# DanecLacey/basic_iterative_solvers

Measured on AMD Instinct MI355X. Metric: CG iterations/sec + SpMV GFLOP/s (% HBM roofline), HPCG 256^3 at 1/2/4/8 GPUs, higher is better.
Workload: dtype f64

## Files before the change

### basic_iterative_solvers_amd/csrc/bis_blas1.hip

```cpp
#include "bis_internal.hpp"

#include <algorithm>
#include <cstdlib>

namespace {

constexpr int kEwThreads = 256;
constexpr int kMaxEwBlocks = 16384;

inline int ew_grid(int64_t n_items) {
    int64_t g = (n_items + kEwThreads - 1) / kEwThreads;
    if (g < 1) g = 1;
    if (g > kMaxDotBlocks) g = kMaxDotBlocks;
    return (int)g;
}
inline int ew_grid_wide(int64_t n_items) {
    int64_t g = (n_items + kEwThreads - 1) / kEwThreads;
    if (g < 1) g = 1;
    if (g > kMaxEwBlocks) g = kMaxEwBlocks;
    return (int)g;
}

typedef double ew_v2d_t __attribute__((ext_vector_type(2)));
__device__ __forceinline__ double2 ld_stream(const double2 *p) {
// ... 180 lines not shown
}

}

bis_status bis_reduce_finish(bis_ctx *ctx, int n_partials, int n_values, size_t stride,
                             double *result_dev) {
    hipLaunchKernelGGL(reduce_finish_kernel, dim3(n_values), dim3(256), 0, ctx->stream,
                       ctx->partials, n_partials, stride, result_dev);
    BIS_HIP_CHECK(ctx, hipGetLastError());
    return BIS_OK;
}

bis_status bis_ensure_partials(bis_ctx *ctx, size_t n) {
    if (n <= ctx->partials_cap) return BIS_OK;
    BIS_HIP_CHECK(ctx, hipStreamSynchronize(ctx->stream));
    if (ctx->partials) BIS_HIP_CHECK(ctx, hipFree(ctx->partials));
    ctx->partials = nullptr;
    ctx->partials_cap = 0;
    BIS_HIP_CHECK(ctx, hipMalloc(&ctx->partials, sizeof(double) * n));
    ctx->partials_cap = n;
    return BIS_OK;
}

bis_status bis_fault_check(bis_ctx *ctx) {
    volatile unsigned *f = ctx->fault_host;
    if (!f || *f == 0) return BIS_OK;
    *f = 0;
    ctx->err = "a triangular sweep lost a hand-off: a row waited for a result that was never published "
               "(a workgroup of the persistent grid could not become resident, or the dependency data is corrupt); "
               "the vectors written since the last blocking call are invalid";
    return BIS_ERR_SYNC;
}

#define BIS_OPTIONS_ENV(X) X(spmv_variant) X(spmv_window) X(spmv_chunk) X(spmv_chunk_fused) X(spmv_xcd_remap) X(trsv_grid) X(ilu0_wgs) X(trsv_wave_wgs) X(trsv_trial) X(trsv_one_xcd) X(trsv_host_analysis) X(ilu0_wave) X(spmv_packed) X(spmv_packed32) X(spmv_valdict) X(spmv_sellwin) X(device_share) X(spmv_sellwin_rows) X(spmv_sellwin_joint) X(spmv_sellwin_pairs) X(spmv_sellwin_masks) X(spmv_colslab) X(spmv_win8) X(spmv_win8_rows) X(spmv_win8_depth) X(spmv_win8_implicit) X(spmv_win8_tune) X(grid_autodetect) X(tune_placement) X(force_rp64) X(trsv_tiled) X(trsv_chain) X(trsv_tile_rows) X(trsv_tile_wgs) X(trsv_tile_edge) X(trsv_tile_backoff)
#define BIS_OPTIONS_API(Y) Y(trsv_batch) Y(trsv_wave) Y(ilu0_persistent) Y(trsv_by_pos) Y(spmv_lds_pad) Y(trsv_chain_idle) Y(trsv_chain_pause) Y(trsv_chain_pairs) Y(trsv_chain_prefix) Y(trsv_tile_exp) Y(cg_nt_x) Y(spmv_sellwin_nt) Y(dist_host_plan) Y(trsv_inject_loss) Y(trsv_inject_oom)

namespace {
std::string &opts_env_seen() { static std::string s; return s; }
std::string upper_env(const char *name) {
    std::string e = "BIS_";
    for (const char *c = name; *c; ++c) e += (char)((*c >= 'a' && *c <= 'z') ? *c - 32 : *c);
    return e;
}
}

bis_options &bis_opts() {
    static bis_options o = [] {
        bis_options v;
#define X(name) { const std::string en = upper_env(#name); if (const char *e = getenv(en.c_str())) { v.name = atoi(e); \
                  std::string &seen = opts_env_seen(); if (!seen.empty()) seen += ' '; seen += en + "=" + e; } }
        BIS_OPTIONS_ENV(X)
#undef X
        return v;
    }();
    return o;
}

extern "C" {

bis_status bis_set_option(const char *name, int value) {
    if (!name) return BIS_ERR_INVALID;
    bis_options &o = bis_opts();
#define X(opt) if (!strcmp(name, #opt)) { o.opt = value; return BIS_OK; }
    BIS_OPTIONS_ENV(X)
    BIS_OPTIONS_API(X)
#undef X
    return BIS_ERR_INVALID;
// ... 377 lines not shown
```

### basic_iterative_solvers_amd/csrc/bis_internal.hpp

```cpp
#pragma once

#include <hip/hip_runtime.h>

#include <cstdint>
#include <cstdio>
#include <cstring>
#include <map>
#include <string>
#include <vector>

#include "bis_hip.h"

struct bis_trsv_plan;

struct bis_named_kernel {
    int type = 0;
    const bis_mat *A = nullptr;
    double *B = nullptr, *C = nullptr;
    int64_t size_B = 0, size_C = 0;
    const double *D = nullptr;
    bool upper = false;
};

struct bis_ctx {
// ... 41 lines not shown
    int trsv_trial = -1;
    int trsv_batch = -1;
    int trsv_by_pos = -1;
    int trsv_one_xcd = -1;
    int tune_placement = -1;
    int spmv_packed32 = -1;
    int spmv_lds_pad = -1;
    int spmv_packed = -1;
    int spmv_valdict = -1;
    int dist_host_plan = -1;
    int grid_autodetect = -1;
    int trsv_chain = -1;
    int trsv_chain_idle = -1;
    int trsv_chain_pause = -1;
    int trsv_chain_prefix = -1;
    int trsv_chain_pairs = -1;
    int trsv_tiled = -1;
    int trsv_tile_rows = -1;
    int trsv_tile_wgs = -1;
    int trsv_tile_backoff = -1;
    int spmv_sellwin_nt = -1;
    int cg_nt_x = -1;
    int trsv_tile_exp = -1;
    int trsv_tile_edge = -1;
    int force_rp64 = -1;
    int spmv_sellwin = -1;
    int spmv_sellwin_rows = -1;
    int spmv_sellwin_pairs = -1;
    int spmv_sellwin_joint = -1;
    int spmv_colslab = -1;
    int spmv_win8 = -1;
    int spmv_win8_rows = -1;
    int spmv_win8_depth = -1;
    int spmv_win8_implicit = -1;
    int spmv_win8_tune = -1;
    int spmv_sellwin_masks = -1;
    int device_share = -1;
    int trsv_inject_oom = -1;
    int trsv_inject_loss = -1;
};
inline bool bis_want_rp64(int64_t nnz) { return nnz >= (int64_t)INT32_MAX - 8 || bis_opts().force_rp64 > 0; }

constexpr int kMaxReduceBlocks = 2048;
constexpr int kMaxDotBlocks = 8192;
constexpr int kWinMaxTiles = 128;
constexpr int kWinTile = 16;
constexpr int kWinTileLog = 4;
constexpr int kSwRows = 256;
constexpr int kSwMaxR = 4;

struct bis_mat {
    int64_t n_rows = 0, n_cols = 0, nnz = 0;
    bool rp64 = false;
    bool view = false;
    void *row_ptr = nullptr;
    int32_t *col = nullptr;
    double *val = nullptr;
    int32_t *blk_row = nullptr;
    int64_t *blk_nnz = nullptr;
    uint16_t *loc = nullptr;
    int32_t *tiles = nullptr;
    int32_t *tile_cnt = nullptr;
    int64_t loc_base = 0;
    int max_tiles = 0;
    bool win_ok = false;
    int n_blocks = 0;
// ... 115 lines not shown
    ++ctx->prof_used;
}

bis_status bis_reduce_finish(bis_ctx *ctx, int n_partials, int n_values,
                             size_t stride, double *result_dev);
bis_status bis_ensure_partials(bis_ctx *ctx, size_t n);
bis_status bis_spmv_launch(bis_ctx *ctx, const bis_mat *A, const double *x,
                           double *y, const double *w, int *n_partials,
                           size_t partials_off = 0);
size_t bis_spmv_partials_bound(const bis_mat *A);
bis_status bis_spmv_trsv_level(bis_ctx *ctx, const bis_mat *T, const double *x, double *y,
                               const double *b, const double *D);
bis_status bis_mat_row_view(bis_ctx *ctx, const bis_mat *A, int64_t ra,
                            int64_t rb, bis_mat **out);

bis_status bis_mat_alloc(bis_ctx *ctx, int64_t n_rows, int64_t n_cols,
                         int64_t nnz, bool rp64, bis_mat **out);
bis_status bis_mat_finalize(bis_ctx *ctx, bis_mat *A);
bis_status bis_spmv_build_window(bis_ctx *ctx, bis_mat *A);
void bis_spmv_drop_packed(bis_mat *A);
void bis_spmv_drop_valdict(bis_mat *A);
bis_status bis_spmv_try_valdict(bis_ctx *ctx, bis_mat *A, bool consecutive_ok);
bis_status bis_spmv_sellwin_try(bis_ctx *ctx, bis_mat *A);
int bis_spmv_sellwin_blocks(const bis_mat *A);
int64_t bis_spmv_sellwin_bytes(const bis_mat *A);
int64_t bis_spmv_sellwin_slices(const bis_mat *A);
int bis_spmv_sellwin_format(const bis_mat *A);
bis_status bis_spmv_sellwin_launch(bis_ctx *ctx, const bis_mat *A, const double *x, double *y, int mode, const double *w,
                                   double *partials, const int *stop, int remap_arg, int grid);
void bis_spmv_sellwin_drop(bis_mat *A);
bis_status bis_spmv_win8_try(bis_ctx *ctx, bis_mat *A);
int bis_spmv_win8_blocks(const bis_mat *A);
int bis_spmv_win8_rows(const bis_mat *A);
int64_t bis_spmv_win8_bytes(const bis_mat *A);
bis_status bis_spmv_win8_launch(bis_ctx *ctx, const bis_mat *A, const double *x, double *y, int mode, const double *w,
                                double *partials, const int *stop, int remap_arg, int grid);
void bis_spmv_win8_drop(bis_mat *A);
bis_status bis_spmv_colslab_build(bis_ctx *ctx, const bis_mat *A, int K, std::vector<bis_mat *> &slabs, bool *ok);
void bis_spmv_colslab_free(bis_ctx *ctx, std::vector<bis_mat *> &slabs);
void bis_spmv_colslab_drop(bis_mat *A);
int bis_spmv_remap_arg(int nb);
int bis_spmv_grid(int nb);
size_t bis_spmv_win8_stream_bytes(const bis_mat *A);
bool bis_spmv_win8_implied(const bis_mat *A);
double bis_spmv_win8_moved_bytes(const bis_mat *A);
bool bis_spmv_win8_fast(const bis_mat *A, double ms);
void *bis_spmv_win8_swap_stream(bis_mat *A, void *stream);
bis_status bis_spmv_try_pack(bis_ctx *ctx, bis_mat *A, int t);
void bis_mat_free_meta(bis_mat *A);
void bis_mat_values_changed(bis_mat *A);
void bis_trsv_plan_destroy(bis_trsv_plan *p);
void bis_trsv_plan_adopt(bis_mat *to, bis_mat *from, bool backward);
bis_status bis_mat_split_strict_impl(bis_ctx *ctx, const bis_mat *A, bis_mat **L_strict,
                                     bis_mat **U_strict, double *D, double *D_inv, bool check_diag);
struct bis_trsv_tiled;
bis_status bis_trsv_tiled_build(bis_ctx *ctx, const bis_mat *T, bool backward, bis_trsv_tiled **out);
bis_status bis_trsv_tiled_solve(bis_ctx *ctx, bis_trsv_tiled *p, double *x, const double *D, const double *b);
void bis_trsv_tiled_destroy(bis_trsv_tiled *p);
bis_status bis_trsv_analyse_device(bis_ctx *ctx, const bis_mat *T, bool backward, int32_t *perm_dev,
                                   std::vector<int64_t> &level_ptr, int &n_levels, int64_t &max_width,
                                   bool &triangular, int **level_out = nullptr);
struct bis_trsv_chain;
bis_status bis_trsv_chain_build(bis_ctx *ctx, const bis_mat *T, bool backward, const int *level_dev, int n_levels,
                                bis_trsv_chain **out);
bis_status bis_trsv_chain_solve(bis_ctx *ctx, const bis_mat *T, bis_trsv_chain *p, double *x, const double *D, const double *b);
void bis_trsv_chain_destroy(bis_trsv_chain *p);
// ... 6 lines not shown
```

### basic_iterative_solvers_amd/csrc/bis_spmv.hip

```cpp
#include "bis_internal.hpp"

#include <algorithm>
#include <cstdlib>
#include <vector>

namespace {

typedef int v4i __attribute__((ext_vector_type(4)));
typedef double v2d __attribute__((ext_vector_type(2)));

typedef unsigned short v4us __attribute__((ext_vector_type(4)));

template <bool WIDE>
__device__ __forceinline__ double x_at(const char *xb, int c) {
    if (WIDE) return *reinterpret_cast<const double *>(xb + (int64_t)c * 8);
    return *reinterpret_cast<const double *>(xb + (uint32_t)((uint32_t)c << 3));
}

constexpr int kPkSegs = 8, kPkOffBits = 13, kPkSpan = 1 << kPkOffBits;
constexpr int kPk3Segs = 32, kPk3OffBits = 11;

template <int PK>
__device__ __forceinline__ int pk_decode(unsigned code, const int (&B)[8], int lane_base, int col_max) {
    int base;
// ... 755 lines not shown
int grid_for_map(int nb, int remap_arg) {
    const int w = remap_arg < -1 ? 8 * -remap_arg : 8;
    return (nb + w - 1) / w * w;
}

int fused_threads(int) { return 256; }

int spmv_variant(const SpmvArgs &a) {
    const int v = bis_opts().spmv_variant >= 0 ? bis_opts().spmv_variant : (a.pk_mode ? 20 : 41);
    return (a.pk_mode >= 2 && v % 10 != 0) ? 20 : v;
}

const char *rowblock_name(int id, const SpmvArgs &a) {
    static const std::vector<std::string> names = [] {
        std::vector<std::string> v;
        for (int u : {1, 2, 4})
            for (int pk = 0; pk < 5; ++pk)
                for (int br = 0; br < 3; ++br)
                    v.push_back("spmv_rowblock_kernel U=" + std::to_string(u) + " PK=" + (pk == 4 ? std::string("0 WIDE") : std::to_string(pk)) +
                                " BR=" + std::to_string(br));
        return v;
    }();
    if (rowblock_is_vd(id, a)) return "spmv_rowblock_vd_kernel";
    const int u = id / 10 == 1 ? 0 : (id / 10 == 2 ? 1 : 2), br = id % 10;
    static const int known[] = {10, 20, 40, 11, 21, 41, 12, 22};
    if (std::find(std::begin(known), std::end(known), id) == std::end(known)) return nullptr;
    const int pk = a.wide ? 4 : a.pk_mode;
    return names[(size_t)(u * 5 + pk) * 3 + br].c_str();
}

const char *form_name(int kind, int v) {
    static const std::vector<std::string> names[3] = {
        [] { std::vector<std::string> n; for (int i = 0; i <= 4; ++i) n.push_back("sellwin fmt=" + std::to_string(i)); return n; }(),
        [] { std::vector<std::string> n; for (int i = 0; i <= 4; ++i) n.push_back("win8 rows=" + std::to_string(i)); return n; }(),
        [] { std::vector<std::string> n; for (int i = 0; i <= 32; ++i) n.push_back("colslab K=" + std::to_string(i)); return n; }()};
    const std::vector<std::string> &t = names[kind];
    return t[(size_t)std::max(0, std::min(v, (int)t.size() - 1))].c_str();
}

}

int spmv_window_mode() { return bis_opts().spmv_window < 0 ? 0 : bis_opts().spmv_window; }

bis_status bis_spmv_build_window(bis_ctx *ctx, bis_mat *A) {
    A->win_ok = false;
    if (!spmv_window_mode() || A->nnz == 0 || A->n_rows == 0) return BIS_OK;
    if ((int64_t)A->chunk_nnz + A->max_row_nnz + 8 > 6144) return BIS_OK;
    const int nb = A->n_blocks;
    int64_t ends[2];
    BIS_HIP_CHECK(ctx, hipMemcpyAsync(&ends[0], A->blk_nnz, 8, hipMemcpyDeviceToHost, ctx->stream));
    BIS_HIP_CHECK(ctx, hipMemcpyAsync(&ends[1], A->blk_nnz + nb, 8, hipMemcpyDeviceToHost, ctx->stream));
    BIS_HIP_CHECK(ctx, hipStreamSynchronize(ctx->stream));
    A->loc_base = ends[0] & ~(int64_t)3;
    const size_t n_loc = (size_t)(ends[1] - A->loc_base) + 16;
    hipFree(A->loc); hipFree(A->tiles); hipFree(A->tile_cnt);
    A->loc = nullptr; A->tiles = nullptr; A->tile_cnt = nullptr;
    BIS_HIP_CHECK(ctx, hipMalloc(&A->loc, sizeof(uint16_t) * n_loc));
    BIS_HIP_CHECK(ctx, hipMalloc(&A->tiles, sizeof(int32_t) * (size_t)nb * kWinMaxTiles));
    BIS_HIP_CHECK(ctx, hipMalloc(&A->tile_cnt, sizeof(int32_t) * (size_t)nb));
    BIS_HIP_CHECK(ctx, hipMemsetAsync(A->loc, 0, sizeof(uint16_t) * n_loc, ctx->stream));
    int *status = (int *)ctx->counters + 40;
    BIS_HIP_CHECK(ctx, hipMemsetAsync(status, 0, 2 * sizeof(int), ctx->stream));
    if (A->rp64)
        hipLaunchKernelGGL(window_build_kernel<int64_t>, dim3(nb), dim3(256), 0, ctx->stream, A->col,
                           A->blk_nnz, nb, A->loc_base, A->loc, A->tiles, A->tile_cnt, status);
    else
        hipLaunchKernelGGL(window_build_kernel<int32_t>, dim3(nb), dim3(256), 0, ctx->stream, A->col,
// ... 378 lines not shown
    }
    if (bis_status st = ensure_packed(ctx, A, use_f ? 1 : 0, &a)) return st;
    if (pass) {
        a.vcode = nullptr;
    } else {
        const int v = bis_opts().spmv_variant;
        const bool lane_per_row = a.vcode && spmv_valdict_mode() >= 2 && (v < 0 || v == 20);
        if (mode != 2 && lane_per_row && bis_opts().spmv_sellwin != 0) {
            if (bis_status st = bis_spmv_sellwin_try(ctx, A)) return st;
            if (const int nb = bis_spmv_sellwin_blocks(A)) {
                block_map(nb);
                p->form = kFormSellwin;
                p->n_partials = mode == 1 ? (int)bis_spmv_sellwin_slices(A) : 0;
                p->name = form_name(0, bis_spmv_sellwin_format(A));
                return BIS_OK;
            }
        }
        if (lane_per_row) {
            if (bis_status st = spmv_try_rowmajor(ctx, A)) return st;
            if (A->rm_state == 1) {
                block_map(A->rm_blocks);
                p->form = kFormRowmajor;
                p->n_partials = mode == 1 ? A->rm_blocks * 4 : 0;
                p->name = "spmv_rowmajor_vd_kernel";
                return BIS_OK;
            }
        }
        if (mode != 2 && !a.vcode && bis_opts().spmv_win8 != 0 && (v < 0 || v == 20)) {
            if (bis_status st = bis_spmv_win8_try(ctx, A)) return st;
            if (const int nb = bis_spmv_win8_blocks(A)) {
                block_map(nb);
                p->form = kFormWin8;
                p->n_partials = mode == 1 ? nb * 4 : 0;
                p->name = form_name(1, bis_spmv_win8_rows(A));
                return BIS_OK;
            }
        }
        if (mode != 2 && !a.vcode && !a.wide && bis_opts().spmv_colslab != 0 && (v < 0 || v == 20 || v == 41)) {
            if (bis_status st = colslab_try(ctx, A, a.pk_mode != 0)) return st;
            if (A->cs_state == 1) {
                p->form = kFormColslab;
                p->n_partials = mode == 1 ? A->colslabs->back()->n_blocks_f * (fused_threads(0) / 64) : 0;
                p->name = form_name(2, (int)A->colslabs->size());
                return BIS_OK;
            }
        }
        if (mode != 2 && bis_opts().spmv_lds_pad > 0) a.lds_bytes += (size_t)bis_opts().spmv_lds_pad;
    }
    const int id = spmv_variant(a);
    p->name = rowblock_name(id, a);
    if (!p->name) { ctx->err = "bis_spmv: unknown BIS_SPMV_VARIANT"; return BIS_ERR_INVALID; }
    p->form = rowblock_is_vd(id, a) ? kFormRowblockVd : kFormRowblock;
    p->n_partials = mode == 1 ? a.nb * (fused_threads(id) / 64) : 0;
    return BIS_OK;
}

static bis_status spmv_launch_plan(bis_ctx *ctx, const bis_mat *A, const SpmvPlan &p) {
    const SpmvArgs &a = p.a;
    switch (p.form) {
    case kFormLongRows: {
        const int grid = (int)std::min<int64_t>((A->n_rows + 3) / 4, 8192);
        if (A->rp64)
            hipLaunchKernelGGL(spmv_wave_per_row_kernel<int64_t>, dim3(grid), dim3(256), 0, ctx->stream,
                               (const int64_t *)A->row_ptr, A->col, A->val, a.x, a.y, A->n_rows);
        else
            hipLaunchKernelGGL(spmv_wave_per_row_kernel<int32_t>, dim3(grid), dim3(256), 0, ctx->stream,
                               (const int32_t *)A->row_ptr, A->col, A->val, a.x, a.y, A->n_rows);
// ... 189 lines not shown
```

### basic_iterative_solvers_amd/csrc/bis_spmv_sell.hip

```cpp
#include <algorithm>
#include <cstring>
#include <cstdio>
#include <cstdlib>
#include <vector>

#include <rocprim/rocprim.hpp>

#include "bis_internal.hpp"

struct bis_sellwin {
    int n_blocks = 0;
    int64_t n_slices = 0, total_chunks = 0;
    int32_t *hdr = nullptr;
    int64_t *slice_chunk0 = nullptr;
    int32_t *own_rank = nullptr;
    uint32_t *codes = nullptr;
    double *dict = nullptr;
    int max_gran = 0;
    int fmt = 0;
    int uniform_chunks = 0;
    int n_pairs = 0, pair_stride = 0, diag_pair = -1;
    int16_t *blk_base = nullptr;
    unsigned long long *pair_key = nullptr;
    uint16_t *row_of = nullptr;
    void *own_codes = nullptr;
    size_t w8_desc = 0, w8_side = 0, w8_end = 0;
    int64_t *slice_rec = nullptr;
    int64_t expl_chunks = 0;
    int64_t win_gran_sum = 0;
    int tune_trials = 0;
    double tune_first_ms = 0.0, tune_kept_ms = 0.0;
    int R = 1;
    bool diag = false;
    int pad_idx = 0, diag_idx = 0;
};

namespace {

constexpr int kSwRuns = 32;
constexpr int kSwRunGran = 64;
constexpr int kSwHash = 4096;
constexpr int kSwMaxGran = 940;
constexpr int kSwDefaultR = 2;
constexpr int kSwMaxPairs = 253;
inline int sw_gran_cap(int R) { return R == 4 ? kSwMaxGran : std::min(kSwMaxGran, (65536 - (4096 + 4096 * R) - 16) / 64); }

__device__ __forceinline__ unsigned long long sw_pair_key(int32_t offset, unsigned vcode) {
    return ((unsigned long long)((unsigned)offset ^ 0x80000000u) << 8) | vcode;
}

__device__ __forceinline__ int sw_wave_max(int v) {
    for (int o = 32; o > 0; o >>= 1) v = max(v, __shfl_xor(v, o));
    return v;
}

template <typename RP>
__global__ __launch_bounds__(256) void sw_plan_kernel(const RP *__restrict__ row_ptr, const int32_t *__restrict__ col,
                                                      int64_t n_rows, int R, int max_gran, int64_t row0, int32_t *__restrict__ hdr,
                                                      int32_t *__restrict__ slice_chunks, int32_t *__restrict__ own_rank, int *status) {
    __shared__ int table[kSwHash];
    __shared__ int list[1024];
// ... 1167 lines not shown
            if ((c_first & 7) == 0 && g0 <= g_first && g_last <= g1) own = rank + (g_first - g0);
            for (int o = 0; o < len && ok; o += kSwRunGran) {
                if (m >= kW8Runs) { ok = false; break; }
                out_g0[m] = g0 + o;
                out_rk[m] = (rank + o) | (min(kSwRunGran, len - o) << 16);
                ++m;
            }
            rank += len;
            if (rank > max_gran) ok = false;
        }
        if (!ok) atomicExch(&failed, 1);
        n_out = m;
        win_gran = rank;
        own_s = own;
    }
    __syncthreads();
    if (failed) {
        if (tid == 0) atomicExch(&status[0], 1);
        return;
    }
    if (tid < 2 * kW8Runs) {
        const int k = tid % kW8Runs;
        int word = 0;
        if (k < n_out) word = tid < kW8Runs ? out_g0[k] : out_rk[k];
        hdr[(size_t)b * 2 * kW8Runs + tid] = word;
    }
    if (tid == 0) {
        own_rank[b] = ident ? own_s : -1;
        atomicMax(&status[1], win_gran);
        atomicAdd(reinterpret_cast<unsigned *>(&status[2]), (unsigned)win_gran);
    }
}

template <typename RP, int PHASE>
__global__ __launch_bounds__(256) void w8_fill_kernel(const RP *__restrict__ row_ptr, const int32_t *__restrict__ col, const double *__restrict__ val,
                                                      int64_t n_rows, int R, const int32_t *__restrict__ hdr,
                                                      const int64_t *__restrict__ slice_chunk0, const uint16_t *__restrict__ row_of,
                                                      unsigned char *__restrict__ stream, int64_t *__restrict__ slice_rec,
                                                      uint2 *__restrict__ desc, unsigned char *__restrict__ side) {
    __shared__ int g0s[kW8Runs], rk[kW8Runs];
    __shared__ int nr_s;
    const int b = blockIdx.x, tid = threadIdx.x, lane = tid & 63, wv = tid >> 6;
    if (tid < kW8Runs) {
        g0s[tid] = hdr[(size_t)b * 2 * kW8Runs + tid];
        const int w2 = hdr[(size_t)b * 2 * kW8Runs + kW8Runs + tid];
        rk[tid] = w2 & 0xffff;
        const unsigned long long m = __ballot((w2 >> 16) != 0);
        if (tid == 0) nr_s = __popcll(m);
    }
    __syncthreads();
    const int nr = nr_s;
    for (int rr = 0; rr < R; ++rr) {
        const int64_t slice = ((int64_t)b * 4 + wv) * R + rr;
        const int64_t pos = slice * 64 + lane;
        const int in_block = row_of[pos];
        const int64_t r = (int64_t)b * kSwRows * R + in_block;
        int64_t rs = 0;
        int len = 0;
        if (r < n_rows) {
            rs = (int64_t)row_ptr[r];
            len = (int)((int64_t)row_ptr[r + 1] - rs);
        }
        const int64_t c0 = slice_chunk0[slice];
        const int nch = (int)(slice_chunk0[slice + 1] - c0);
        bool implicit = false;
        if (PHASE == 1) implicit = __ballot(r < n_rows && len == __builtin_amdgcn_readfirstlane(len)) == ~0ull;
// ... 50 lines not shown
    const unsigned char *p = stream + (size_t)c * kW8ChunkBytes;
    W8Chunk ch;
    ch.code = __builtin_nontemporal_load(reinterpret_cast<const w8_v2u *>(p + lane * 8));
    ch.v0 = __builtin_nontemporal_load(reinterpret_cast<const w8_v2d *>(p + 512 + lane * 16));
    ch.v1 = __builtin_nontemporal_load(reinterpret_cast<const w8_v2d *>(p + 1536 + lane * 16));
    return ch;
}

__device__ __forceinline__ void w8_load_values(const unsigned char *__restrict__ stream, int64_t c, int lane, W8Chunk &ch) {
    const unsigned char *p = stream + (size_t)c * kW8ValBytes;
    ch.v0 = __builtin_nontemporal_load(reinterpret_cast<const w8_v2d *>(p + lane * 16));
    ch.v1 = __builtin_nontemporal_load(reinterpret_cast<const w8_v2d *>(p + 1024 + lane * 16));
}

typedef unsigned short w8_v2h __attribute__((ext_vector_type(2)));
__device__ __forceinline__ unsigned w8_imply(unsigned code, unsigned off2) {
    const unsigned pad = (code & 0x10001u) * 0xffffu;
    return __builtin_bit_cast(unsigned, __builtin_bit_cast(w8_v2h, code) + __builtin_bit_cast(w8_v2h, off2)) & ~pad;
}

__device__ __forceinline__ void w8_consume(const unsigned char *win, const W8Chunk &ch, double &acc) {
#pragma clang fp contract(off)
    const double x0 = *reinterpret_cast<const double *>(win + (ch.code.x & 0xffffu));
    const double x1 = *reinterpret_cast<const double *>(win + (ch.code.x >> 16));
    const double x2 = *reinterpret_cast<const double *>(win + (ch.code.y & 0xffffu));
    const double x3 = *reinterpret_cast<const double *>(win + (ch.code.y >> 16));
    const double p0 = ch.v0.x * x0, p1 = ch.v0.y * x1, p2 = ch.v1.x * x2, p3 = ch.v1.y * x3;
    acc = acc + p0;
    acc = acc + p1;
    acc = acc + p2;
    acc = acc + p3;
}

template <int MODE, int R, int D, bool IMPL>
__global__ __launch_bounds__(256) void spmv_win8_kernel(
    const double *x, double *__restrict__ y, int64_t n_rows, int64_t n_cols, int n_blocks, int remap_arg, const double *w,
    double *__restrict__ partials, const int *stop, const int32_t *__restrict__ hdr, const int64_t *__restrict__ slice_chunk0,
    const unsigned char *__restrict__ stream, int x_al16, const int32_t *__restrict__ own_rank, const uint16_t *__restrict__ row_of,
    const w8_v2u *__restrict__ desc, const unsigned char *__restrict__ side, const int64_t *__restrict__ slice_rec) {
    if (stop && stop[1]) return;
    extern __shared__ __attribute__((aligned(16))) unsigned char lds[];
    const int b = remap_arg > 0 ? xcd_remap(blockIdx.x, remap_arg)
                                : (remap_arg < -1 ? xcd_group_remap(blockIdx.x, -remap_arg) : (int)blockIdx.x);
    if (b >= n_blocks) return;
    const int tid = threadIdx.x, lane = tid & 63;
    const int wv = __builtin_amdgcn_readfirstlane(tid >> 6);
    const int hw_g = hdr[(size_t)b * 2 * kW8Runs + lane], hw_r = hdr[(size_t)b * 2 * kW8Runs + kW8Runs + lane];
    const int64_t slice0 = ((int64_t)b * 4 + wv) * R;
    const int64_t block_row0 = (int64_t)b * kSwRows * R;
    int64_t rows_of[R];
#pragma unroll
    for (int r = 0; r < R; ++r) rows_of[r] = block_row0 + row_of[(slice0 + r) * 64 + lane];
    const int64_t my_bnd = slice_chunk0[slice0 + min(lane, R)];
    auto bnd = [&](int r) {
        const unsigned lo = (unsigned)__builtin_amdgcn_readlane((int)(unsigned)(unsigned long long)my_bnd, r);
        const unsigned hi = (unsigned)__builtin_amdgcn_readlane((int)(unsigned)((unsigned long long)my_bnd >> 32), r);
        return (int64_t)(((unsigned long long)hi << 32) | lo);
    };
    const int64_t C0 = bnd(0), C1 = bnd(R);
    const int64_t c_last = max(C1 - 1, C0);
    int64_t e[R];
#pragma unroll
    for (int rr = 0; rr < R; ++rr) e[rr] = bnd(rr + 1);
    int64_t rec[R + 1];
    unsigned off2[R];
    if (IMPL) {
        const int64_t my_rec = slice_rec[slice0 + min(lane, R)];
#pragma unroll
        for (int r = 0; r <= R; ++r) {
            const unsigned lo = (unsigned)__builtin_amdgcn_readlane((int)(unsigned)(unsigned long long)my_rec, r);
            const unsigned hi = (unsigned)__builtin_amdgcn_readlane((int)(unsigned)((unsigned long long)my_rec >> 32), r);
            rec[r] = (int64_t)(((unsigned long long)hi << 32) | lo);
        }
#pragma unroll
        for (int r = 0; r < R; ++r) off2[r] = rec[r + 1] == rec[r] ? (unsigned)(rows_of[r] - block_row0) * 0x80008u : 0u;
    }
    auto load = [&](int64_t cc) {
        if (!IMPL) return w8_load(stream, cc, lane);
        W8Chunk ch;
        w8_load_values(stream, cc, lane, ch);
        int64_t rs = 0, re = 0, cs = 0;
#pragma unroll
        for (int rr = 0; rr < R; ++rr)
            if (cc >= (rr ? e[rr - 1] : C0) && cc < e[rr]) { rs = rec[rr]; re = rec[rr + 1]; cs = rr ? e[rr - 1] : C0; }
        if (re > rs) ch.code = __builtin_nontemporal_load(reinterpret_cast<const w8_v2u *>(side + (size_t)(rs + cc - cs) * 512 + lane * 8));
        else ch.code = desc[cc];
        return ch;
    };
    W8Chunk ring[D];
#pragma unroll
    for (int d = 0; d < D; ++d) ring[d] = load(min(C0 + d, c_last));
    double wr[R];
    int own = -1;
    if (MODE == 1 && own_rank) own = own_rank[b];
#pragma unroll
    for (int r = 0; r < R; ++r) {
        const int64_t row = rows_of[r];
        wr[r] = (MODE == 1 && own < 0 && row < n_rows) ? w[row] : 0.0;
    }
    if (tid == 0) *reinterpret_cast<double *>(lds) = -0.0;
    {
        const int n_runs = __popcll(__ballot((hw_r >> 16) != 0));
        unsigned char *win = lds + 16;
        for (int k = 0; k < n_runs; ++k) {
            const int g0 = __builtin_amdgcn_readlane(hw_g, k);
            const int w2 = __builtin_amdgcn_readlane(hw_r, k);
            const int rank = w2 & 0xffff, n_pieces = (w2 >> 16) * 4;
            const int j = (wv + k) & 3;
            const int p = j * 64 + lane;
            const int64_t c = (int64_t)g0 * 8 + 2 * p;
            unsigned char *dst = win + (size_t)rank * 64 + (size_t)j * 1024;
            if (p < n_pieces) {
                if (x_al16 && c + 1 < n_cols) {
                    __builtin_amdgcn_global_load_lds((const __attribute__((address_space(1))) void *)(x + c),
                                                     (__attribute__((address_space(3))) void *)dst, 16, 0, 0);
                } else {
                    double2 v;
                    v.x = c < n_cols ? x[c] : 0.0;
                    v.y = c + 1 < n_cols ? x[c + 1] : 0.0;
                    *reinterpret_cast<double2 *>(dst + lane * 16) = v;
                }
            }
        }
    }
    __syncthreads();
    if (MODE == 1 && own >= 0) {
#pragma unroll
        for (int r = 0; r < R; ++r) wr[r] = *reinterpret_cast<const double *>(lds + 16 + ((size_t)own * 8 + (wv * R + r) * 64 + lane) * 8);
    }
    double dot_acc = 0.0;
    int64_t c = C0;
    int next = 0;
    double acc = 0.0;
    unsigned cur_off = IMPL ? off2[0] : 0u;
#define W8_END_SLICES()                                                                    \
    _Pragma("unroll") for (int rr = 0; rr < R; ++rr)                                       \
        if (rr == next && c == e[rr]) {                                                    \
            const int64_t row = rows_of[rr];                                               \
            if (row < n_rows) y[row] = acc;                                                \
            if (MODE == 1) dot_acc += row < n_rows ? acc * wr[rr] : 0.0;                   \
            acc = 0.0;                                                                     \
            ++next;                                                                        \
            if (IMPL) cur_off = off2[rr + 1 < R ? rr + 1 : R - 1];                         \
        }
    W8_END_SLICES()
    while (c < C1) {
#pragma unroll
        for (int d = 0; d < D; ++d) {
            if (c < C1) {
                W8Chunk cur = ring[d];
                ring[d] = load(min(c + D, c_last));
                if (IMPL) {
                    cur.code.x = w8_imply(cur.code.x, cur_off);
                    cur.code.y = w8_imply(cur.code.y, cur_off);
                }
                w8_consume(lds, cur, acc);
                ++c;
                W8_END_SLICES()
            }
        }
    }
#undef W8_END_SLICES
    if (MODE == 1) {
        const double t = wave_sum(dot_acc);
        if (lane == 0) partials[(size_t)b * 4 + wv] = t;
    }
}

}

void bis_spmv_win8_drop(bis_mat *A) {
    if (A->sw8) {
        if (A->sw8->own_codes) A->sw8->codes = reinterpret_cast<uint32_t *>(A->sw8->own_codes);
        hipFree(A->sw8->hdr); hipFree(A->sw8->slice_chunk0); hipFree(A->sw8->own_rank); hipFree(A->sw8->codes); hipFree(A->sw8->row_of);
        hipFree(A->sw8->slice_rec);
        delete A->sw8;
        A->sw8 = nullptr;
    }
    A->sw8_state = 0;
}

int bis_spmv_win8_blocks(const bis_mat *A) { return A->sw8_state == 1 ? A->sw8->n_blocks : 0; }
int bis_spmv_win8_rows(const bis_mat *A) { return A->sw8_state == 1 ? A->sw8->R : 0; }
bool bis_spmv_win8_implied(const bis_mat *A) { return A->sw8_state == 1 && A->sw8->slice_rec != nullptr; }
int64_t bis_spmv_win8_bytes(const bis_mat *A) {
    if (A->sw8_state != 1) return 0;
    const bis_sellwin *sw = A->sw8;
    const int64_t meta = (int64_t)sw->n_blocks * (8 * kW8Runs + 2 * kSwRows * sw->R) + 8 * (sw->n_slices + 1);
    if (!bis_spmv_win8_implied(A)) return sw->total_chunks * (int64_t)kW8ChunkBytes + meta;
    return sw->total_chunks * (int64_t)kW8ValBytes + 8 * (sw->total_chunks - sw->expl_chunks) + 512 * sw->expl_chunks + meta + 8 * (sw->n_slices + 1);
}

size_t bis_spmv_win8_stream_bytes(const bis_mat *A) {
    if (A->sw8_state != 1) return 0;
    return bis_spmv_win8_implied(A) ? A->sw8->w8_end : (size_t)kW8ChunkBytes * (size_t)(A->sw8->total_chunks + 1);
// ... 123 lines not shown
    if (A->n_rows == 0 || A->nnz == 0 || A->n_cols >= ((int64_t)1 << 31) - 16) return BIS_OK;
    int R = bis_opts().spmv_win8_rows > 0 ? std::min(bis_opts().spmv_win8_rows, 4) : 4;
    if (R == 3) R = 2;
    while (R > 1 && A->n_rows < (int64_t)kSwRows * R * 1024) R >>= 1;
    for (;; R >>= 1) {
        bool too_large = false;
        if (bis_status st = w8_try_rows(ctx, A, R, &too_large)) return st;
        if (A->sw8_state == 1 || !too_large || R == 1 || bis_opts().spmv_win8_rows > 0) return BIS_OK;
        A->sw8_state = -1;
    }
}

static bis_status w8_try_rows(bis_ctx *ctx, bis_mat *A, int R, bool *window_too_large) {
    *window_too_large = false;
    const int64_t nb64 = (A->n_rows + (int64_t)kSwRows * R - 1) / ((int64_t)kSwRows * R);
    if (nb64 > (int64_t)1 << 26) return BIS_OK;
    const int nb = (int)nb64;
    bis_sellwin *sw = new bis_sellwin;
    A->sw8 = sw;
    sw->n_blocks = nb;
    sw->R = R;
    sw->n_slices = (int64_t)nb * 4 * R;
    sw->fmt = 5;
    int32_t *slice_chunks = nullptr;
    void *tmp = nullptr;
    int *status = (int *)ctx->counters + 52;
    W8_CHECK(hipMalloc(&sw->hdr, sizeof(int32_t) * 2 * kW8Runs * (size_t)nb));
    W8_CHECK(hipMalloc(&sw->own_rank, sizeof(int32_t) * (size_t)nb));
    W8_CHECK(hipMemsetAsync(sw->own_rank, 0xFF, sizeof(int32_t) * (size_t)nb, ctx->stream));
    W8_CHECK(hipMalloc(&sw->row_of, sizeof(uint16_t) * (size_t)nb * kSwRows * (size_t)R));
    W8_CHECK(hipMalloc(&slice_chunks, sizeof(int32_t) * (size_t)(sw->n_slices + 1)));
    W8_CHECK(hipMalloc(&sw->slice_chunk0, sizeof(int64_t) * (size_t)(sw->n_slices + 1)));
    W8_CHECK(hipMemsetAsync(status, 0, 3 * sizeof(int), ctx->stream));
    W8_CHECK(hipMemsetAsync(status + 5, 0, sizeof(int), ctx->stream));
    W8_CHECK(hipMemsetAsync(slice_chunks, 0, sizeof(int32_t) * (size_t)(sw->n_slices + 1), ctx->stream));
    W8_CHECK(hipMemsetAsync(sw->hdr, 0, sizeof(int32_t) * 2 * kW8Runs * (size_t)nb, ctx->stream));
    if (A->rp64) hipLaunchKernelGGL(w8_plan_kernel<int64_t>, dim3(nb), dim3(256), 0, ctx->stream, (const int64_t *)A->row_ptr, A->col, A->n_rows, R, kSwMaxGran, A->view_row0, sw->hdr, slice_chunks, sw->own_rank, sw->row_of, status);
    else hipLaunchKernelGGL(w8_plan_kernel<int32_t>, dim3(nb), dim3(256), 0, ctx->stream, (const int32_t *)A->row_ptr, A->col, A->n_rows, R, kSwMaxGran, A->view_row0, sw->hdr, slice_chunks, sw->own_rank, sw->row_of, status);
    W8_CHECK(hipGetLastError());
    int h[3] = {0, 0, 0};
    W8_CHECK(hipMemcpyAsync(h, status, sizeof h, hipMemcpyDeviceToHost, ctx->stream));
    const int64_t ns1 = sw->n_slices + 1;
    hipLaunchKernelGGL(sw_widen_kernel, dim3((unsigned)((ns1 + 255) / 256)), dim3(256), 0, ctx->stream, slice_chunks, sw->slice_chunk0, ns1);
    W8_CHECK(hipGetLastError());
    size_t tmp_bytes = 0;
    W8_CHECK(rocprim::exclusive_scan(nullptr, tmp_bytes, sw->slice_chunk0, sw->slice_chunk0, (int64_t)0, (size_t)ns1, rocprim::plus<int64_t>(), ctx->stream));
    W8_CHECK(hipMalloc(&tmp, tmp_bytes));
    W8_CHECK(rocprim::exclusive_scan(tmp, tmp_bytes, sw->slice_chunk0, sw->slice_chunk0, (int64_t)0, (size_t)ns1, rocprim::plus<int64_t>(), ctx->stream));
    int64_t total = 0;
    W8_CHECK(hipMemcpyAsync(&total, sw->slice_chunk0 + sw->n_slices, sizeof total, hipMemcpyDeviceToHost, ctx->stream));
    W8_CHECK(hipStreamSynchronize(ctx->stream));
    hipFree(tmp); tmp = nullptr;
    hipFree(slice_chunks); slice_chunks = nullptr;
    sw->total_chunks = total;
    sw->max_gran = h[1];
    sw->win_gran_sum = (int64_t)(unsigned)h[2];
    if (h[0] || (double)total * 256.0 > 1.12 * (double)A->nnz + 256.0 * 4 * 64) {
        if (getenv("BIS_WIN8_STATS")) fprintf(stderr, "win8 plan (R = %d): %s, %.1f %% padding: not used\n", R, h[0] ? "window not representable" : "representable", 100.0 * ((double)total * 256.0 / (double)A->nnz - 1.0));
        *window_too_large = h[0] != 0;
        bis_spmv_win8_drop(A);
        A->sw8_state = -1;
        return BIS_OK;
    }
#define W8_FILL(PHASE, STREAM, DESC, SIDE)                                                                                                        \
    do {                                                                                                                                          \
        if (A->rp64) hipLaunchKernelGGL((w8_fill_kernel<int64_t, PHASE>), dim3(nb), dim3(256), 0, ctx->stream, (const int64_t *)A->row_ptr, A->col, \
                                        A->val, A->n_rows, R, sw->hdr, sw->slice_chunk0, sw->row_of, STREAM, sw->slice_rec, DESC, SIDE);           \
        else hipLaunchKernelGGL((w8_fill_kernel<int32_t, PHASE>), dim3(nb), dim3(256), 0, ctx->stream, (const int32_t *)A->row_ptr, A->col,     \
                                A->val, A->n_rows, R, sw->hdr, sw->slice_chunk0, sw->row_of, STREAM, sw->slice_rec, DESC, SIDE);                   \
        W8_CHECK(hipGetLastError());                                                                                                              \
    } while (0)
    sw->expl_chunks = total;
    if (bis_opts().spmv_win8_implicit != 0 && total > 0) {
        W8_CHECK(hipMalloc(&sw->slice_rec, sizeof(int64_t) * (size_t)ns1));
        W8_CHECK(hipMemsetAsync(sw->slice_rec, 0, sizeof(int64_t) * (size_t)ns1, ctx->stream));
        W8_FILL(1, nullptr, nullptr, nullptr);
        tmp_bytes = 0;
        W8_CHECK(rocprim::exclusive_scan(nullptr, tmp_bytes, sw->slice_rec, sw->slice_rec, (int64_t)0, (size_t)ns1, rocprim::plus<int64_t>(), ctx->stream));
        W8_CHECK(hipMalloc(&tmp, tmp_bytes));
        W8_CHECK(rocprim::exclusive_scan(tmp, tmp_bytes, sw->slice_rec, sw->slice_rec, (int64_t)0, (size_t)ns1, rocprim::plus<int64_t>(), ctx->stream));
        int64_t expl = 0;
        W8_CHECK(hipMemcpyAsync(&expl, sw->slice_rec + sw->n_slices, sizeof expl, hipMemcpyDeviceToHost, ctx->stream));
        W8_CHECK(hipStreamSynchronize(ctx->stream));
        hipFree(tmp); tmp = nullptr;
        if (2 * (total - expl) >= total) sw->expl_chunks = expl;
        else { hipFree(sw->slice_rec); sw->slice_rec = nullptr; }
    }
    unsigned char *stream = nullptr;
    const size_t chunk_bytes = sw->slice_rec ? kW8ValBytes : kW8ChunkBytes;
    size_t stream_bytes = chunk_bytes * (size_t)(total + 1);
    if (sw->slice_rec) {
        sw->w8_desc = stream_bytes;
        sw->w8_side = sw->w8_desc + ((8 * (size_t)(total + 1) + 255) & ~(size_t)255);
        sw->w8_end = stream_bytes = sw->w8_side + 512 * (size_t)sw->expl_chunks;
    }
    W8_CHECK(hipMalloc(&stream, stream_bytes));
    sw->codes = reinterpret_cast<uint32_t *>(stream);
    W8_CHECK(hipMemsetAsync(stream + (size_t)total * chunk_bytes, 0, chunk_bytes, ctx->stream));
    if (sw->slice_rec) {
        W8_CHECK(hipMemsetAsync(stream + sw->w8_desc, 0, sw->w8_side - sw->w8_desc, ctx->stream));
        W8_FILL(2, stream, reinterpret_cast<uint2 *>(stream + sw->w8_desc), stream + sw->w8_side);
    } else {
        W8_FILL(0, stream, nullptr, nullptr);
    }
#undef W8_FILL
    A->sw8_state = 1;
    if (bis_status tst = w8_tune_placement(ctx, A)) return tst;
    if (getenv("BIS_WIN8_STATS")) fprintf(stderr, "win8 plan (R = %d): %d blocks, window <= %d granules (%zu bytes), %.1f %% padding: used; implied slots: %s, %.1f %% of %lld chunks implicit; stream at %p (%zu bytes), hdr %p\n", R, nb, sw->max_gran, (size_t)(2 + 8 * sw->max_gran) * 8, 100.0 * ((double)total * 256.0 / (double)A->nnz - 1.0), sw->slice_rec ? "built" : "not built", 100.0 * (double)(total - sw->expl_chunks) / (double)std::max<int64_t>(total, 1), (long long)total, (void *)sw->codes, bis_spmv_win8_stream_bytes(A), (void *)sw->hdr);
    return BIS_OK;
}
#undef W8_CHECK

bis_status bis_spmv_win8_launch(bis_ctx *ctx, const bis_mat *A, const double *x, double *y, int mode, const double *w,
                                double *partials, const int *stop, int remap_arg, int grid) {
    const bis_sellwin *sw = A->sw8;
    const int x_al16 = ((uintptr_t)x & 15) == 0;
    const size_t lds = (size_t)(2 + 8 * sw->max_gran) * 8;
    const unsigned char *stream = reinterpret_cast<const unsigned char *>(sw->codes);
    const int32_t *own = (mode == 1 && w == x + A->view_row0 && x_al16) ? sw->own_rank : nullptr;
    const bool ragged = (double)sw->total_chunks * 256.0 > 1.08 * (double)A->nnz;
    const int depth = bis_opts().spmv_win8_depth > 0 ? bis_opts().spmv_win8_depth : (sw->R == 4 ? (ragged ? 2 : 1) : 3);
#define W8_L3(MODE, RR, DD) do { if (sw->slice_rec) W8_L4(MODE, RR, DD, true); else W8_L4(MODE, RR, DD, false); } while (0)
#define W8_L4(MODE, RR, DD, IMPL) hipLaunchKernelGGL((spmv_win8_kernel<MODE, RR, DD, IMPL>), dim3(grid), dim3(256), lds, ctx->stream, x, y, A->n_rows, A->n_cols, \
                                               sw->n_blocks, remap_arg, w, partials, stop, sw->hdr, sw->slice_chunk0, stream, x_al16, own, sw->row_of, \
                                               reinterpret_cast<const w8_v2u *>(stream + sw->w8_desc), stream + sw->w8_side, sw->slice_rec)
#define W8_L2(MODE, RR) do { if (depth <= 1) W8_L3(MODE, RR, 1); else if (depth == 2) W8_L3(MODE, RR, 2); else if (depth == 3) W8_L3(MODE, RR, 3); else if (depth <= 5) W8_L3(MODE, RR, 4); else W8_L3(MODE, RR, 6); } while (0)
#define W8_L1(MODE) do { if (sw->R == 4) W8_L2(MODE, 4); else if (sw->R == 2) W8_L2(MODE, 2); else W8_L2(MODE, 1); } while (0)
    if (mode == 1) W8_L1(1); else W8_L1(0);
#undef W8_L1
#undef W8_L2
#undef W8_L3
#undef W8_L4
    BIS_HIP_CHECK(ctx, hipGetLastError());
    return BIS_OK;
}
```

Measured before the change: 1139.

## Add straight-line pipelined win8 SpMV walk for uniform seven-chunk slices

Adds a fully unrolled straight-line path to the win8 SpMV kernel for blocks where every slice holds exactly seven chunks, a case detected at plan time by a new counting kernel. The path prefetches chunks through a deeper software pipeline (depth 4 by default) and drops the per-chunk slice-end bookkeeping of the generic ring loop. It is on by default when at least 90% of slices are uniform and the implied-slot layout exists, which fits HPCG 27-point stencils. In exchange it adds kernel instantiations and register pressure, plus an extra plan-time kernel and copy.

Result: no change. 1137 (-0.1%).

```diff
diff --git a/basic_iterative_solvers_amd/csrc/bis_blas1.hip b/basic_iterative_solvers_amd/csrc/bis_blas1.hip
--- a/basic_iterative_solvers_amd/csrc/bis_blas1.hip
+++ b/basic_iterative_solvers_amd/csrc/bis_blas1.hip
@@ -236,7 +236,7 @@
     return BIS_ERR_SYNC;
 }
 
-#define BIS_OPTIONS_ENV(X) X(spmv_variant) X(spmv_window) X(spmv_chunk) X(spmv_chunk_fused) X(spmv_xcd_remap) X(trsv_grid) X(ilu0_wgs) X(trsv_wave_wgs) X(trsv_trial) X(trsv_one_xcd) X(trsv_host_analysis) X(ilu0_wave) X(spmv_packed) X(spmv_packed32) X(spmv_valdict) X(spmv_sellwin) X(device_share) X(spmv_sellwin_rows) X(spmv_sellwin_joint) X(spmv_sellwin_pairs) X(spmv_sellwin_masks) X(spmv_colslab) X(spmv_win8) X(spmv_win8_rows) X(spmv_win8_depth) X(spmv_win8_implicit) X(spmv_win8_tune) X(grid_autodetect) X(tune_placement) X(force_rp64) X(trsv_tiled) X(trsv_chain) X(trsv_tile_rows) X(trsv_tile_wgs) X(trsv_tile_edge) X(trsv_tile_backoff)
+#define BIS_OPTIONS_ENV(X) X(spmv_variant) X(spmv_window) X(spmv_chunk) X(spmv_chunk_fused) X(spmv_xcd_remap) X(trsv_grid) X(ilu0_wgs) X(trsv_wave_wgs) X(trsv_trial) X(trsv_one_xcd) X(trsv_host_analysis) X(ilu0_wave) X(spmv_packed) X(spmv_packed32) X(spmv_valdict) X(spmv_sellwin) X(device_share) X(spmv_sellwin_rows) X(spmv_sellwin_joint) X(spmv_sellwin_pairs) X(spmv_sellwin_masks) X(spmv_colslab) X(spmv_win8) X(spmv_win8_rows) X(spmv_win8_depth) X(spmv_win8_pipe) X(spmv_win8_implicit) X(spmv_win8_tune) X(grid_autodetect) X(tune_placement) X(force_rp64) X(trsv_tiled) X(trsv_chain) X(trsv_tile_rows) X(trsv_tile_wgs) X(trsv_tile_edge) X(trsv_tile_backoff)
 #define BIS_OPTIONS_API(Y) Y(trsv_batch) Y(trsv_wave) Y(ilu0_persistent) Y(trsv_by_pos) Y(spmv_lds_pad) Y(trsv_chain_idle) Y(trsv_chain_pause) Y(trsv_chain_pairs) Y(trsv_chain_prefix) Y(trsv_tile_exp) Y(cg_nt_x) Y(spmv_sellwin_nt) Y(dist_host_plan) Y(trsv_inject_loss) Y(trsv_inject_oom)
 
 namespace {
diff --git a/basic_iterative_solvers_amd/csrc/bis_internal.hpp b/basic_iterative_solvers_amd/csrc/bis_internal.hpp
--- a/basic_iterative_solvers_amd/csrc/bis_internal.hpp
+++ b/basic_iterative_solvers_amd/csrc/bis_internal.hpp
@@ -97,6 +97,7 @@
     int spmv_win8 = -1;
     int spmv_win8_rows = -1;
     int spmv_win8_depth = -1;
+    int spmv_win8_pipe = -1;
     int spmv_win8_implicit = -1;
     int spmv_win8_tune = -1;
     int spmv_sellwin_masks = -1;
@@ -278,6 +279,7 @@
 bis_status bis_spmv_win8_try(bis_ctx *ctx, bis_mat *A);
 int bis_spmv_win8_blocks(const bis_mat *A);
 int bis_spmv_win8_rows(const bis_mat *A);
+const char *bis_spmv_win8_name(const bis_mat *A);
 int64_t bis_spmv_win8_bytes(const bis_mat *A);
 bis_status bis_spmv_win8_launch(bis_ctx *ctx, const bis_mat *A, const double *x, double *y, int mode, const double *w,
                                 double *partials, const int *stop, int remap_arg, int grid);
diff --git a/basic_iterative_solvers_amd/csrc/bis_spmv.hip b/basic_iterative_solvers_amd/csrc/bis_spmv.hip
--- a/basic_iterative_solvers_amd/csrc/bis_spmv.hip
+++ b/basic_iterative_solvers_amd/csrc/bis_spmv.hip
@@ -811,7 +811,7 @@
 const char *form_name(int kind, int v) {
     static const std::vector<std::string> names[3] = {
         [] { std::vector<std::string> n; for (int i = 0; i <= 4; ++i) n.push_back("sellwin fmt=" + std::to_string(i)); return n; }(),
-        [] { std::vector<std::string> n; for (int i = 0; i <= 4; ++i) n.push_back("win8 rows=" + std::to_string(i)); return n; }(),
+        {},
         [] { std::vector<std::string> n; for (int i = 0; i <= 32; ++i) n.push_back("colslab K=" + std::to_string(i)); return n; }()};
     const std::vector<std::string> &t = names[kind];
     return t[(size_t)std::max(0, std::min(v, (int)t.size() - 1))].c_str();
@@ -1256,7 +1256,7 @@
                 block_map(nb);
                 p->form = kFormWin8;
                 p->n_partials = mode == 1 ? nb * 4 : 0;
-                p->name = form_name(1, bis_spmv_win8_rows(A));
+                p->name = bis_spmv_win8_name(A);
                 return BIS_OK;
             }
         }
diff --git a/basic_iterative_solvers_amd/csrc/bis_spmv_sell.hip b/basic_iterative_solvers_amd/csrc/bis_spmv_sell.hip
--- a/basic_iterative_solvers_amd/csrc/bis_spmv_sell.hip
+++ b/basic_iterative_solvers_amd/csrc/bis_spmv_sell.hip
@@ -27,6 +27,7 @@
     size_t w8_desc = 0, w8_side = 0, w8_end = 0;
     int64_t *slice_rec = nullptr;
     int64_t expl_chunks = 0;
+    int uni_nch = 0;
     int64_t win_gran_sum = 0;
     int tune_trials = 0;
     double tune_first_ms = 0.0, tune_kept_ms = 0.0;
@@ -1260,6 +1261,12 @@
     }
 }
 
+__global__ __launch_bounds__(256) void w8_count_kernel(const int32_t *__restrict__ slice_chunks, int64_t n_slices, int *status) {
+    const int64_t i = (int64_t)blockIdx.x * 256 + threadIdx.x;
+    const unsigned long long m = __ballot(i < n_slices && slice_chunks[i < n_slices ? i : 0] == status[5]);
+    if ((threadIdx.x & 63) == 0 && m) atomicAdd(&status[6], __popcll(m));
+}
+
 template <typename RP, int PHASE>
 __global__ __launch_bounds__(256) void w8_fill_kernel(const RP *__restrict__ row_ptr, const int32_t *__restrict__ col, const double *__restrict__ val,
                                                       int64_t n_rows, int R, const int32_t *__restrict__ hdr,
@@ -1376,7 +1383,12 @@
     acc = acc + p3;
 }
 
-template <int MODE, int R, int D, bool IMPL>
+__device__ __forceinline__ double w8_mul(double a, double b) {
+#pragma clang fp contract(off)
+    return a * b;
+}
+
+template <int MODE, int R, int D, bool IMPL, int NCH = 0>
 __global__ __launch_bounds__(256) void spmv_win8_kernel(
     const double *x, double *__restrict__ y, int64_t n_rows, int64_t n_cols, int n_blocks, int remap_arg, const double *w,
     double *__restrict__ partials, const int *stop, const int32_t *__restrict__ hdr, const int64_t *__restrict__ slice_chunk0,
@@ -1431,9 +1443,34 @@
         else ch.code = desc[cc];
         return ch;
     };
-    W8Chunk ring[D];
-#pragma unroll
-    for (int d = 0; d < D; ++d) ring[d] = load(min(C0 + d, c_last));
+    static_assert(NCH == 0 || IMPL, "the straight-line walk reads the implied-slot layout");
+    constexpr int DG = NCH ? (R == 4 ? 1 : 3) : D;
+    constexpr int NP = NCH ? D : 1, KP = R * NCH, NC1 = NCH ? NCH : 1;
+    bool uni = false;
+    if constexpr (NCH > 0) {
+        uni = block_row0 + (int64_t)kSwRows * R <= n_rows;
+#pragma unroll
+        for (int rr = 0; rr < R; ++rr) uni = uni && e[rr] - (rr ? e[rr - 1] : C0) == NCH;
+    }
+    auto pload = [&](int k) {
+        W8Chunk ch;
+        if constexpr (NCH > 0) {
+            const int rr = k / NCH, j = k % NCH;
+            w8_load_values(stream, C0 + k, lane, ch);
+            const unsigned char *p = rec[rr + 1] == rec[rr] ? reinterpret_cast<const unsigned char *>(desc + (C0 + k))
+                                                            : side + (size_t)(rec[rr] + j) * 512 + lane * 8;
+            ch.code = *reinterpret_cast<const w8_v2u *>(p);
+        }
+        return ch;
+    };
+    W8Chunk ring[DG], pring[NP];
+    if (uni) {
+#pragma unroll
+        for (int d = 0; d < NP; ++d) if (d < KP) pring[d] = pload(d);
+    } else {
+#pragma unroll
+        for (int d = 0; d < DG; ++d) ring[d] = load(min(C0 + d, c_last));
+    }
     double wr[R];
     int own = -1;
     if (MODE == 1 && own_rank) own = own_rank[b];
@@ -1473,9 +1510,26 @@
         for (int r = 0; r < R; ++r) wr[r] = *reinterpret_cast<const double *>(lds + 16 + ((size_t)own * 8 + (wv * R + r) * 64 + lane) * 8);
     }
     double dot_acc = 0.0;
+    double acc = 0.0;
+    if (uni) {
+#pragma unroll
+        for (int k = 0; k < KP; ++k) {
+            const int rr = k / NC1;
+            W8Chunk cur = pring[k % NP];
+            if (k + NP < KP) pring[k % NP] = pload(k + NP);
+            __builtin_amdgcn_sched_barrier(0);
+            cur.code.x = w8_imply(cur.code.x, off2[rr]);
+            cur.code.y = w8_imply(cur.code.y, off2[rr]);
+            w8_consume(lds, cur, acc);
+            if (k % NC1 == NC1 - 1) {
+                y[rows_of[rr]] = acc;
+                if (MODE == 1) dot_acc += w8_mul(acc, wr[rr]);
+                acc = 0.0;
+            }
+        }
+    } else {
     int64_t c = C0;
     int next = 0;
-    double acc = 0.0;
     unsigned cur_off = IMPL ? off2[0] : 0u;
 #define W8_END_SLICES()                                                                    \
     _Pragma("unroll") for (int rr = 0; rr < R; ++rr)                                       \
@@ -1490,10 +1544,10 @@
     W8_END_SLICES()
     while (c < C1) {
 #pragma unroll
-        for (int d = 0; d < D; ++d) {
+        for (int d = 0; d < DG; ++d) {
             if (c < C1) {
                 W8Chunk cur = ring[d];
-                ring[d] = load(min(c + D, c_last));
+                ring[d] = load(min(c + DG, c_last));
                 if (IMPL) {
                     cur.code.x = w8_imply(cur.code.x, cur_off);
                     cur.code.y = w8_imply(cur.code.y, cur_off);
@@ -1505,6 +1559,7 @@
         }
     }
 #undef W8_END_SLICES
+    }
     if (MODE == 1) {
         const double t = wave_sum(dot_acc);
         if (lane == 0) partials[(size_t)b * 4 + wv] = t;
@@ -1694,14 +1749,17 @@
     W8_CHECK(hipMalloc(&slice_chunks, sizeof(int32_t) * (size_t)(sw->n_slices + 1)));
     W8_CHECK(hipMalloc(&sw->slice_chunk0, sizeof(int64_t) * (size_t)(sw->n_slices + 1)));
     W8_CHECK(hipMemsetAsync(status, 0, 3 * sizeof(int), ctx->stream));
-    W8_CHECK(hipMemsetAsync(status + 5, 0, sizeof(int), ctx->stream));
+    W8_CHECK(hipMemsetAsync(status + 5, 0, 2 * sizeof(int), ctx->stream));
     W8_CHECK(hipMemsetAsync(slice_chunks, 0, sizeof(int32_t) * (size_t)(sw->n_slices + 1), ctx->stream));
     W8_CHECK(hipMemsetAsync(sw->hdr, 0, sizeof(int32_t) * 2 * kW8Runs * (size_t)nb, ctx->stream));
     if (A->rp64) hipLaunchKernelGGL(w8_plan_kernel<int64_t>, dim3(nb), dim3(256), 0, ctx->stream, (const int64_t *)A->row_ptr, A->col, A->n_rows, R, kSwMaxGran, A->view_row0, sw->hdr, slice_chunks, sw->own_rank, sw->row_of, status);
     else hipLaunchKernelGGL(w8_plan_kernel<int32_t>, dim3(nb), dim3(256), 0, ctx->stream, (const int32_t *)A->row_ptr, A->col, A->n_rows, R, kSwMaxGran, A->view_row0, sw->hdr, slice_chunks, sw->own_rank, sw->row_of, status);
     W8_CHECK(hipGetLastError());
-    int h[3] = {0, 0, 0};
+    int h[3] = {0, 0, 0}, h_uni[2] = {0, 0};
     W8_CHECK(hipMemcpyAsync(h, status, sizeof h, hipMemcpyDeviceToHost, ctx->stream));
+    hipLaunchKernelGGL(w8_count_kernel, dim3((unsigned)((sw->n_slices + 255) / 256)), dim3(256), 0, ctx->stream, slice_chunks, sw->n_slices, status);
+    W8_CHECK(hipGetLastError());
+    W8_CHECK(hipMemcpyAsync(h_uni, status + 5, sizeof h_uni, hipMemcpyDeviceToHost, ctx->stream));
     const int64_t ns1 = sw->n_slices + 1;
     hipLaunchKernelGGL(sw_widen_kernel, dim3((unsigned)((ns1 + 255) / 256)), dim3(256), 0, ctx->stream, slice_chunks, sw->slice_chunk0, ns1);
     W8_CHECK(hipGetLastError());
@@ -1717,6 +1775,7 @@
     sw->total_chunks = total;
     sw->max_gran = h[1];
     sw->win_gran_sum = (int64_t)(unsigned)h[2];
+    sw->uni_nch = 10 * (int64_t)h_uni[1] >= 9 * sw->n_slices ? h_uni[0] : 0;
     if (h[0] || (double)total * 256.0 > 1.12 * (double)A->nnz + 256.0 * 4 * 64) {
         if (getenv("BIS_WIN8_STATS")) fprintf(stderr, "win8 plan (R = %d): %s, %.1f %% padding: not used\n", R, h[0] ? "window not representable" : "representable", 100.0 * ((double)total * 256.0 / (double)A->nnz - 1.0));
         *window_too_large = h[0] != 0;
@@ -1773,6 +1832,29 @@
 }
 #undef W8_CHECK
 
+constexpr int kW8PipeDepth = 4;
+static void w8_instance(const bis_mat *A, int *depth, int *nch) {
+    const bis_sellwin *sw = A->sw8;
+    *nch = (bis_opts().spmv_win8_pipe != 0 && sw->slice_rec && sw->uni_nch == 7) ? 7 : 0;
+    const bool ragged = (double)sw->total_chunks * 256.0 > 1.08 * (double)A->nnz;
+    const int d = bis_opts().spmv_win8_depth > 0 ? bis_opts().spmv_win8_depth : (*nch ? kW8PipeDepth : (sw->R == 4 ? (ragged ? 2 : 1) : 3));
+    *depth = d <= 1 ? 1 : (d <= 3 ? d : (d <= 5 ? 4 : 6));
+}
+
+const char *bis_spmv_win8_name(const bis_mat *A) {
+    static const std::vector<std::string> names = [] {
+        std::vector<std::string> n;
+        for (int r = 0; r <= 4; ++r)
+            for (int d = 0; d <= 6; ++d)
+                for (int p : {0, 7}) n.push_back("win8 rows=" + std::to_string(r) + " depth=" + std::to_string(d) + " pipe=" + std::to_string(p));
+        return n;
+    }();
+    if (A->sw8_state != 1) return "";
+    int depth = 0, nch = 0;
+    w8_instance(A, &depth, &nch);
+    return names[(size_t)((std::max(0, std::min(A->sw8->R, 4)) * 7 + depth) * 2 + (nch ? 1 : 0))].c_str();
+}
+
 bis_status bis_spmv_win8_launch(bis_ctx *ctx, const bis_mat *A, const double *x, double *y, int mode, const double *w,
                                 double *partials, const int *stop, int remap_arg, int grid) {
     const bis_sellwin *sw = A->sw8;
@@ -1780,13 +1862,13 @@
     const size_t lds = (size_t)(2 + 8 * sw->max_gran) * 8;
     const unsigned char *stream = reinterpret_cast<const unsigned char *>(sw->codes);
     const int32_t *own = (mode == 1 && w == x + A->view_row0 && x_al16) ? sw->own_rank : nullptr;
-    const bool ragged = (double)sw->total_chunks * 256.0 > 1.08 * (double)A->nnz;
-    const int depth = bis_opts().spmv_win8_depth > 0 ? bis_opts().spmv_win8_depth : (sw->R == 4 ? (ragged ? 2 : 1) : 3);
-#define W8_L3(MODE, RR, DD) do { if (sw->slice_rec) W8_L4(MODE, RR, DD, true); else W8_L4(MODE, RR, DD, false); } while (0)
-#define W8_L4(MODE, RR, DD, IMPL) hipLaunchKernelGGL((spmv_win8_kernel<MODE, RR, DD, IMPL>), dim3(grid), dim3(256), lds, ctx->stream, x, y, A->n_rows, A->n_cols, \
+    int depth = 0, nch = 0;
+    w8_instance(A, &depth, &nch);
+#define W8_L3(MODE, RR, DD) do { if (nch) W8_L4(MODE, RR, DD, true, 7); else if (sw->slice_rec) W8_L4(MODE, RR, DD, true, 0); else W8_L4(MODE, RR, DD, false, 0); } while (0)
+#define W8_L4(MODE, RR, DD, IMPL, NCH) hipLaunchKernelGGL((spmv_win8_kernel<MODE, RR, DD, IMPL, NCH>), dim3(grid), dim3(256), lds, ctx->stream, x, y, A->n_rows, A->n_cols, \
                                                sw->n_blocks, remap_arg, w, partials, stop, sw->hdr, sw->slice_chunk0, stream, x_al16, own, sw->row_of, \
                                                reinterpret_cast<const w8_v2u *>(stream + sw->w8_desc), stream + sw->w8_side, sw->slice_rec)
-#define W8_L2(MODE, RR) do { if (depth <= 1) W8_L3(MODE, RR, 1); else if (depth == 2) W8_L3(MODE, RR, 2); else if (depth == 3) W8_L3(MODE, RR, 3); else if (depth <= 5) W8_L3(MODE, RR, 4); else W8_L3(MODE, RR, 6); } while (0)
+#define W8_L2(MODE, RR) do { if (depth == 1) W8_L3(MODE, RR, 1); else if (depth == 2) W8_L3(MODE, RR, 2); else if (depth == 3) W8_L3(MODE, RR, 3); else if (depth == 4) W8_L3(MODE, RR, 4); else W8_L3(MODE, RR, 6); } while (0)
 #define W8_L1(MODE) do { if (sw->R == 4) W8_L2(MODE, 4); else if (sw->R == 2) W8_L2(MODE, 2); else W8_L2(MODE, 1); } while (0)
     if (mode == 1) W8_L1(1); else W8_L1(0);
 #undef W8_L1
```
